# apple/ml-hugs

Hardware: AMD Instinct MI355X
Metric: rasterizer fwd+bwd FPS @1080p vs #Gaussians; achieved HBM GB/s vs peak (higher is better)
Workload: dtype f32

## Files before the change

### ml-hugs_amd/csrc/blend.hip

```cpp
#include <cstdlib>

#include "hgs_common.h"
#include "blend_fwd.h"

namespace hgs {

__global__ void __launch_bounds__(256)
blend_forward_kernel(Camera cam, uint32_t lastg, const uint2* __restrict__ ranges, const uint64_t* __restrict__ act,
                     size_t act_stride, const uint32_t* __restrict__ act_count, const Splat* __restrict__ splats, const float* __restrict__ bg, float* __restrict__ out_color,
                     float* __restrict__ final_T, uint32_t* __restrict__ n_contrib, const uint32_t* __restrict__ n_total,
                     int clamp_output, const uint32_t* __restrict__ large_tiles, uint32_t num_workers, int long_sorted, Ckpt ck)
{
    __shared__ DeepShared deep;
    if (((const_u32p)n_total)[1]) return;
    const uint32_t deep_min = num_workers != 0u ? ((const_u32p)n_total)[8] : 0u;
    const bool deep_blend = deep_min != 0u;
    if (blockIdx.x < num_workers) {
        if (deep_blend)
            deep_forward_worker(blockIdx.x, num_workers, cam, lastg, ranges, act, act_stride, act_count, splats, bg, out_color, final_T,
                                n_contrib, clamp_output, ck, large_tiles, n_total, deep, gridDim.x == num_workers);
        if (gridDim.x != num_workers) return;
        const uint32_t count = ((const_u32p)n_total)[2], threshold = ((const_u32p)n_total)[4];
        const int w = __builtin_amdgcn_readfirstlane(threadIdx.x >> 6);
        for (uint32_t li = blockIdx.x; li < count; li += num_workers) {
            const uint32_t tile = ((const_u32p)large_tiles)[li];
            const v2u range = ((const_u2p)ranges)[tile];
            const uint32_t n_tile = range.y - range.x;
            if (n_tile <= threshold || (deep_blend && n_tile > deep_min)) continue;
            float4* ck_tile = ckpt_begin(ck, tile, n_tile);
            blend_forward_wave(cam, lastg, (int)(tile % (uint32_t)cam.gx), (int)(tile / (uint32_t)cam.gx), w,
                               ((const_u32p)act_count)[tile * NUM_LISTS + w], act + (size_t)w * act_stride + range.x, splats, bg, out_color,
                               final_T, n_contrib, clamp_output, ck_tile, ck.quad_nproc + tile * 4u + (uint32_t)w);
        }
        return;
    }
    const int w = __builtin_amdgcn_readfirstlane(threadIdx.x >> 6);
    const int tile = (int)(blockIdx.x - num_workers);
    const v2u range = ((const_u2p)ranges)[tile];
    const uint32_t n_tile = range.y > range.x ? range.y - range.x : 0u;
    if (n_tile > ((const_u32p)n_total)[4]) {
        if (!long_sorted) return;
        if (deep_blend && n_tile > deep_min) {
            ckpt_begin(ck, (uint32_t)tile, n_tile);
            return;
        }
    }
    else if (long_sorted == 2) return;
    const uint32_t n = n_tile ? ((const_u32p)act_count)[tile * NUM_LISTS + w] : 0u;
    float4* ck_tile = ckpt_begin(ck, (uint32_t)tile, n_tile);
    blend_forward_wave(cam, lastg, tile % cam.gx, tile / cam.gx, w, n, act + (size_t)w * act_stride + range.x, splats, bg, out_color,
                       final_T, n_contrib, clamp_output, ck_tile, ck.quad_nproc + (uint32_t)tile * 4u + (uint32_t)w);
}

void launch_blend_forward(const Camera& cam, int P, const uint2* ranges, const uint64_t* act, size_t act_stride,
                          const uint32_t* act_count, const Splat* splats, const float* bg, float* out_color,
                          float* final_T, uint32_t* n_contrib, const uint32_t* n_total, bool clamp_output,
                          const uint32_t* large_tiles, bool all_tiles, bool long_sorted, const Ckpt& ck, hipStream_t st)
{
    const int tiles = cam.gx * cam.gy;
    const bool deep = deep_forward_enabled();
    const uint32_t workers = long_sorted && deep ? deep_workers_for(tiles) : 0u;
    if (!all_tiles && !deep) {
        hipLaunchKernelGGL(blend_forward_kernel, dim3(tiles), dim3(256), 0, st, cam, (uint32_t)(P - 1), ranges, act, act_stride, act_count,
                           splats, bg, out_color, final_T, n_contrib, n_total, clamp_output ? 1 : 0, large_tiles, 0u, 2, ck);
        return;
    }
    if (workers + (all_tiles ? tiles : 0) == 0) return;
    hipLaunchKernelGGL(blend_forward_kernel, dim3(workers + (all_tiles ? tiles : 0)), dim3(256), 0, st, cam, (uint32_t)(P - 1),
                       ranges, act, act_stride, act_count, splats, bg, out_color, final_T, n_contrib, n_total, clamp_output ? 1 : 0,
                       large_tiles, workers, long_sorted ? 1 : 0, ck);
}

template <int CTRL>
__device__ __forceinline__ float dpp_mov(float v)
{
    return __builtin_bit_cast(float, __builtin_amdgcn_update_dpp(0, __builtin_bit_cast(int, v), CTRL, 0xf, 0xf, true));
}
constexpr int DPP_QUAD_XOR1 = 0xB1;
constexpr int DPP_QUAD_XOR2 = 0x4E;
constexpr int DPP_ROW_ROR8 = 0x128;
constexpr int DPP_ROW_MIRROR = 0x140;
constexpr int DPP_ROW_HALF_MIRROR = 0x141;

typedef uint32_t swap_pair_t __attribute__((ext_vector_type(2)));
template <int W>
__device__ __forceinline__ float swap_add(float a, float b)
{
    const uint32_t ua = __builtin_bit_cast(uint32_t, a), ub = __builtin_bit_cast(uint32_t, b);
    swap_pair_t r;
    if constexpr (W == 32) r = __builtin_amdgcn_permlane32_swap(ua, ub, false, false);
    else r = __builtin_amdgcn_permlane16_swap(ua, ub, false, false);
    const uint32_t r0 = r.x, r1 = r.y;
    return __builtin_bit_cast(float, r0) + __builtin_bit_cast(float, r1);
}

template <int CTRL>
__device__ __forceinline__ float pair_step(float a, float b, bool hi)
{
    const float keep = hi ? b : a, send = hi ? a : b;
    return keep + dpp_mov<CTRL>(send);
}

struct PixBwd {
    float pxf, pyf;
    float T;
    float S;
    float g0, g1, g2;
    uint32_t last_contributor;
};

__device__ __forceinline__ unsigned long long bwd_pixel(const SplatRec& s, uint32_t pos1, PixBwd& p, float dy, float bdy,
                                                        float q, float (&v)[9])
{
    const float dx = s.x - p.pxf;
    const float t = __builtin_fmaf(s.A, dx, bdy);
    const float e = __builtin_fmaf(-t, t, q);
    const float alpha_uncapped = __builtin_amdgcn_exp2f(e);
    const float alpha = fminf(ALPHA_MAX, alpha_uncapped);
    float alpha_if_reached = pos1 <= p.last_contributor ? alpha : 0.0f;
    asm("" : "+v"(alpha_if_reached));
    const bool act_lane = alpha_if_reached >= ALPHA_MIN;
    const unsigned long long took = __builtin_amdgcn_ballot_w64(act_lane);
    if (act_lane) {
        const float inv = __builtin_amdgcn_rcpf(1.0f - alpha);
        p.T = p.T * inv;
        const float cg = __builtin_fmaf(s.r, p.g0, __builtin_fmaf(s.g, p.g1, s.b * p.g2));
        const float dL_dalpha = __builtin_fmaf(p.T, cg, -(p.S * inv));
        const float dch = alpha * p.T;
        p.S = __builtin_fmaf(cg, dch, p.S);
        const float u = alpha_uncapped * dL_dalpha;
        const float ux = u * dx, uy = u * dy;
        v[0] += ux;
        v[1] += uy;
        v[2] = __builtin_fmaf(ux, dx, v[2]);
        v[3] = __builtin_fmaf(ux, dy, v[3]);
        v[4] = __builtin_fmaf(uy, dy, v[4]);
        v[5] += u;
        v[6] = __builtin_fmaf(dch, p.g0, v[6]);
        v[7] = __builtin_fmaf(dch, p.g1, v[7]);
        v[8] = __builtin_fmaf(dch, p.g2, v[8]);
    }
    return took;
}

struct BwdSegment {
    uint32_t lo, hi;
    const float4* start;
    const float4* end_state;
};

template <int NQ, bool SEG = false>
__device__ __forceinline__ void
blend_backward_wave(const Camera& cam, uint32_t lastg, int tile, int w, v2u range, const uint64_t* __restrict__ act,
                    size_t act_stride, const uint32_t* __restrict__ act_count, const Splat* __restrict__ splats,
                    const float* __restrict__ bg, const float* __restrict__ final_T, const uint32_t* __restrict__ n_contrib,
                    const float* __restrict__ dL_dpix, float* __restrict__ grad_accum, const BwdSegment seg = BwdSegment{})
{
    static_assert(!SEG || NQ == 1, "segments are per quad");
    const int lane = threadIdx.x & 63;
    const int tx = tile % cam.gx, ty = tile / cam.gx;
    const int list_id = NQ == 4 ? 4 : w;
    const size_t HW = (size_t)cam.H * cam.W;
    const float bg0 = bg[0], bg1 = bg[1], bg2 = bg[2];

    PixBwd p[NQ];
    uint32_t wmax = 0;
    float ld_T[NQ], ld_g[NQ][3];
    uint32_t ld_n[NQ];
    bool in_img[NQ];
#pragma unroll
    for (int k = 0; k < NQ; ++k) {
        const int quad = NQ == 4 ? k : w;
        const int px = tx * TILE + (quad & 1) * 8 + (lane & 7);
        const int py = ty * TILE + (quad >> 1) * 8 + (lane >> 3);
        in_img[k] = px < cam.W && py < cam.H;
        const size_t pix = in_img[k] ? (size_t)py * cam.W + px : 0;
        p[k].pxf = (float)px, p[k].pyf = (float)py;
        ld_T[k] = final_T[pix], ld_n[k] = n_contrib[pix];
        ld_g[k][0] = dL_dpix[pix], ld_g[k][1] = dL_dpix[HW + pix], ld_g[k][2] = dL_dpix[2 * HW + pix];
    }
    float4 ck_start = make_float4(0.f, 0.f, 0.f, 0.f), ck_end = ck_start;
    if (SEG && seg.start) ck_start = seg.start[lane], ck_end = seg.end_state[lane];
#pragma unroll
    for (int k = 0; k < NQ; ++k) {
        const float Tf = in_img[k] ? ld_T[k] : 0.0f;
        p[k].T = Tf;
        p[k].g0 = in_img[k] && (ld_n[k] >> 29 & 1u) ? ld_g[k][0] : 0.0f;
        p[k].g1 = in_img[k] && (ld_n[k] >> 30 & 1u) ? ld_g[k][1] : 0.0f;
        p[k].g2 = in_img[k] && (ld_n[k] >> 31 & 1u) ? ld_g[k][2] : 0.0f;
        p[k].S = Tf * (bg0 * p[k].g0 + bg1 * p[k].g1 + bg2 * p[k].g2);
        if (SEG && seg.start) {
            p[k].T = __builtin_fabsf(ck_start.x);
            p[k].S = __builtin_fmaf(p[k].g0, ck_end.y - ck_start.y,
                                    __builtin_fmaf(p[k].g1, ck_end.z - ck_start.z, __builtin_fmaf(p[k].g2, ck_end.w - ck_start.w, p[k].S)));
        }
        p[k].last_contributor = in_img[k] ? (ld_n[k] & 0x0FFFFFFFu) : 0u;
        wmax = max(wmax, p[k].last_contributor);
    }
#pragma unroll
    for (int d = 32; d >= 1; d >>= 1) wmax = max(wmax, (uint32_t)__shfl_xor((int)wmax, d, 64));
    wmax = __builtin_amdgcn_readfirstlane(wmax);
    if (wmax == 0) return;
    const bool b3 = lane & 8;
    const int half_row = lane >> 3;
    const int slot_in_row[4] = {0, 2, 1, 3};
    const int slot_of_lane = lane == 63 ? 8 : ((lane & 7) == 0 ? slot_in_row[half_row >> 1] + 4 * (half_row & 1) : -1);

    uint32_t n = SEG ? seg.hi - seg.lo : ((const_u32p)act_count)[tile * NUM_LISTS + list_id];
    if (n == 0) return;
    const uint64_t* first = act + (size_t)list_id * act_stride + range.x + (SEG ? seg.lo : 0u);
    if (SEG && (uint32_t)(((const_u64p)first)[0] >> 32) > wmax) return;
    if ((uint32_t)(((const_u64p)first)[n - 1] >> 32) > wmax) {
        uint32_t lo = 0, hi = n - 1;
        while (lo < hi) {
            const uint32_t mid = (lo + hi) >> 1;
            if ((uint32_t)(((const_u64p)first)[mid] >> 32) <= wmax) lo = mid + 1; else hi = mid;
        }
        n = lo;
        if (n == 0) return;
    }
    const uint64_t* top = first + n;

    auto backward_entry = [&](const SplatRec& s, uint32_t val, uint32_t pos1) {
        if (pos1 > wmax) return;
        float v[9] = {0.f, 0.f, 0.f, 0.f, 0.f, 0.f, 0.f, 0.f, 0.f};
        unsigned long long took = 0ull;
        if constexpr (NQ == 4) {
#pragma unroll
            for (int r = 0; r < 2; ++r) {
                if (((val >> (GID_BITS + 2 * r)) & 3u) == 0u) continue;
                const float dy = s.y - p[2 * r].pyf, bdy = s.B * dy, cdy = s.C * dy, q = __builtin_fmaf(-cdy, cdy, s.L);
                if ((val >> (GID_BITS + 2 * r)) & 1u) took |= bwd_pixel(s, pos1, p[2 * r], dy, bdy, q, v);
                if ((val >> (GID_BITS + 2 * r + 1)) & 1u) took |= bwd_pixel(s, pos1, p[2 * r + 1], dy, bdy, q, v);
            }
        } else {
            const float dy = s.y - p[0].pyf, bdy = s.B * dy, cdy = s.C * dy, q = __builtin_fmaf(-cdy, cdy, s.L);
            took = bwd_pixel(s, pos1, p[0], dy, bdy, q, v);
        }
        if (took == 0ull) return;
        const float s0 = swap_add<32>(v[0], v[1]), s1 = swap_add<32>(v[2], v[3]);
        const float s2 = swap_add<32>(v[4], v[5]), s3 = swap_add<32>(v[6], v[7]);
        const float t0 = swap_add<16>(s0, s1), t1 = swap_add<16>(s2, s3);
        float y = pair_step<DPP_ROW_ROR8>(t0, t1, b3);
        y += dpp_mov<DPP_ROW_HALF_MIRROR>(y);
        y += dpp_mov<DPP_QUAD_XOR2>(y);
        y += dpp_mov<DPP_QUAD_XOR1>(y);
        float vb = v[8] + dpp_mov<DPP_QUAD_XOR1>(v[8]);
        vb += dpp_mov<DPP_QUAD_XOR2>(vb);
        vb += dpp_mov<DPP_ROW_HALF_MIRROR>(vb);
        vb += dpp_mov<DPP_ROW_MIRROR>(vb);
        asm("s_nop 1\n\tv_add_f32_dpp %0, %0, %0 row_bcast:15 row_mask:0xa bank_mask:0xf" : "+v"(vb));
        asm("s_nop 1\n\tv_add_f32_dpp %0, %0, %0 row_bcast:31 row_mask:0xc bank_mask:0xf" : "+v"(vb));
        if (slot_of_lane >= 0) atomicAdd(grad_accum + (size_t)(val & GID_MASK) * 12u + slot_of_lane, lane == 63 ? vb : y);
    };

    v4u eA = load_pair(top - 2, 0);
    SplatRec rA0 = load_rec(splats, eA.z, lastg), rA1 = load_rec(splats, eA.x, lastg);
    v4u eB = load_pair(top - 4, 0);
    for (uint32_t j = 0; j < n; j += 4) {
        __builtin_amdgcn_s_waitcnt(0xC07F);
        const SplatRec rB0 = load_rec(splats, eB.z, lastg), rB1 = load_rec(splats, eB.x, lastg);
        const v4u eA2 = load_pair(top - 6 - j, 0);
        backward_entry(rA0, eA.z, eA.w);
        if (j + 1 < n) backward_entry(rA1, eA.x, eA.y);
        if (j + 2 >= n) break;
        rA0 = load_rec(splats, eA2.z, lastg), rA1 = load_rec(splats, eA2.x, lastg);
        const v4u eB2 = load_pair(top - 8 - j, 0);
        backward_entry(rB0, eB.z, eB.w);
        if (j + 3 < n) backward_entry(rB1, eB.x, eB.y);
        eA = eA2, eB = eB2;
    }
}

template <int NQ>
__global__ void __launch_bounds__(256)
blend_backward_kernel(Camera cam, uint32_t lastg, const uint2* __restrict__ ranges, const uint64_t* __restrict__ act,
                      size_t act_stride, const uint32_t* __restrict__ act_count, const Splat* __restrict__ splats,
                      const float* __restrict__ bg, const float* __restrict__ final_T, const uint32_t* __restrict__ n_contrib,
                      const float* __restrict__ dL_dpix, float* __restrict__ grad_accum, uint32_t skip_from)
{
    const int num_tiles = cam.gx * cam.gy;
    const int w = __builtin_amdgcn_readfirstlane(threadIdx.x >> 6);
    const int vbid = NQ == 1 ? (int)blockIdx.x : (int)blockIdx.x * 4 + w;
    if (vbid >= num_tiles) return;
    const int tile = vbid;
    const v2u range = ((const_u2p)ranges)[tile];
    if (range.y <= range.x) return;
    if (skip_from && range.y - range.x >= skip_from) return;
    blend_backward_wave<NQ>(cam, lastg, tile, w, range, act, act_stride, act_count, splats, bg, final_T, n_contrib, dL_dpix, grad_accum);
}

__device__ __forceinline__ void
blend_backward_slot(uint32_t slot, const Camera& cam, uint32_t lastg, const uint2* __restrict__ ranges, const uint64_t* __restrict__ act,
                    size_t act_stride, const Splat* __restrict__ splats, const float* __restrict__ bg, const float* __restrict__ final_T,
                    const uint32_t* __restrict__ n_contrib, const float* __restrict__ dL_dpix, float* __restrict__ grad_accum, const Ckpt& ck)
{
    const int w = __builtin_amdgcn_readfirstlane(threadIdx.x >> 6);
    if (slot >= ((const_u32p)ck.seg_first)[cam.gx * cam.gy]) return;
    const uint32_t tile = ((const_u32p)ck.slot_tile)[slot];
    if (tile == CKPT_SLOT_NONE) return;
    const uint32_t first_slot = ((const_u32p)ck.seg_first)[tile];
    const uint32_t m = slot - first_slot;
    const uint32_t walked = ((const_u32p)ck.quad_nproc)[tile * 4u + (uint32_t)w];
    const uint32_t segs = (walked + (uint32_t)(CKPT_SEG - 1)) >> CKPT_SHIFT;
    if (m >= segs) return;
    const v2u range = ((const_u2p)ranges)[tile];
    BwdSegment seg;
    seg.lo = m << CKPT_SHIFT, seg.hi = min(walked, (m + 1u) << CKPT_SHIFT);
    seg.start = m + 1u < segs ? ck.state + (size_t)(first_slot + m) * 256u + w * 64 : nullptr;
    seg.end_state = ck.state + (size_t)(first_slot + segs - 1u) * 256u + w * 64;
    blend_backward_wave<1, true>(cam, lastg, (int)tile, w, range, act, act_stride, nullptr, splats, bg, final_T, n_contrib, dL_dpix,
                                 grad_accum, seg);
}

__global__ void __launch_bounds__(256)
blend_backward_segmented_kernel(Camera cam, uint32_t lastg, const uint2* __restrict__ ranges, const uint64_t* __restrict__ act,
                                size_t act_stride, const Splat* __restrict__ splats, const float* __restrict__ bg,
                                const float* __restrict__ final_T, const uint32_t* __restrict__ n_contrib,
                                const float* __restrict__ dL_dpix, float* __restrict__ grad_accum, Ckpt ck)
{
    blend_backward_slot(blockIdx.x, cam, lastg, ranges, act, act_stride, splats, bg, final_T, n_contrib, dL_dpix, grad_accum, ck);
}

#ifndef HGS_MIXED_ATTR
#define HGS_MIXED_ATTR
#endif
__global__ void __launch_bounds__(256) HGS_MIXED_ATTR
blend_backward_mixed_kernel(Camera cam, uint32_t lastg, const uint2* __restrict__ ranges, const uint64_t* __restrict__ act,
                            size_t act_stride, const uint32_t* __restrict__ act_count, const Splat* __restrict__ splats,
                            const float* __restrict__ bg, const float* __restrict__ final_T, const uint32_t* __restrict__ n_contrib,
                            const float* __restrict__ dL_dpix, float* __restrict__ grad_accum, Ckpt ck, uint32_t dense_blocks)
{
    if (blockIdx.x >= dense_blocks) {
        blend_backward_slot(blockIdx.x - dense_blocks, cam, lastg, ranges, act, act_stride, splats, bg, final_T, n_contrib, dL_dpix,
                            grad_accum, ck);
        return;
    }
    const int w = __builtin_amdgcn_readfirstlane(threadIdx.x >> 6);
    const int tile = (int)blockIdx.x * 4 + w;
    if (tile >= cam.gx * cam.gy) return;
    const v2u range = ((const_u2p)ranges)[tile];
    if (range.y <= range.x || range.y - range.x >= CKPT_DEEP_MIN) return;
    blend_backward_wave<4>(cam, lastg, tile, w, range, act, act_stride, act_count, splats, bg, final_T, n_contrib, dL_dpix, grad_accum);
}

void launch_blend_backward(const Camera& cam, int P, const uint2* ranges, const uint64_t* act, size_t act_stride,
                           const uint32_t* act_count, bool sparse_frame, const Splat* splats, const float* bg,
                           const float* final_T, const uint32_t* n_contrib, const float* dL_dpix, float* grad_accum,
                           const Ckpt& ck, int64_t num_rendered, int64_t dense_slots, hipStream_t st)
{
    const int num_tiles = cam.gx * cam.gy;
    const int force = switches().bwd_waves_per_tile;
    const bool per_quad = force ? force == 4 : sparse_frame;
    if (ck.state) {
        uint32_t slots = (uint32_t)(num_rendered >> CKPT_SHIFT) + (uint32_t)num_tiles;
        if (!sparse_frame && dense_slots >= 0 && (uint64_t)dense_slots < slots) slots = (uint32_t)dense_slots;
        const bool two_launches = switches().bwd_two_launches;
        if ((sparse_frame || two_launches) && slots)
            hipLaunchKernelGGL(blend_backward_segmented_kernel, dim3(slots), dim3(256), 0, st, cam, (uint32_t)(P - 1), ranges, act,
                               act_stride, splats, bg, final_T, n_contrib, dL_dpix, grad_accum, ck);
        if (!sparse_frame && two_launches)
            hipLaunchKernelGGL(blend_backward_kernel<4>, dim3((num_tiles + 3) / 4), dim3(256), 0, st, cam, (uint32_t)(P - 1), ranges,
                               act, act_stride, act_count, splats, bg, final_T, n_contrib, dL_dpix, grad_accum, CKPT_DEEP_MIN);
        else if (!sparse_frame) {
            const uint32_t dense_blocks = (uint32_t)(num_tiles + 3) / 4u;
            hipLaunchKernelGGL(blend_backward_mixed_kernel, dim3(dense_blocks + slots), dim3(256), 0, st, cam, (uint32_t)(P - 1), ranges,
                               act, act_stride, act_count, splats, bg, final_T, n_contrib, dL_dpix, grad_accum, ck, dense_blocks);
        }
    } else if (per_quad)
        hipLaunchKernelGGL(blend_backward_kernel<1>, dim3(num_tiles), dim3(256), 0, st, cam, (uint32_t)(P - 1), ranges, act,
                           act_stride, act_count, splats, bg, final_T, n_contrib, dL_dpix, grad_accum, 0u);
    else
        hipLaunchKernelGGL(blend_backward_kernel<4>, dim3((num_tiles + 3) / 4), dim3(256), 0, st, cam, (uint32_t)(P - 1), ranges,
                           act, act_stride, act_count, splats, bg, final_T, n_contrib, dL_dpix, grad_accum, 0u);
}

}
```

Measured before the change: 2126.

## Replace permlane/DPP gradient reduction with per-wave LDS transpose reduction

Each backward entry now writes its eight per-lane gradient partials into a per-wave LDS buffer and reads them back transposed as two float4s, then finishes with three DPP steps. This replaces the earlier permlane32/16 swap-and-DPP butterfly. Two splats are staged into separate buffers before reading, so their reductions can interleave. The change adds 16 KB of shared memory per block plus wave barriers and fences, which may reduce occupancy and adds LDS traffic.

```diff
diff --git a/ml-hugs_amd/csrc/blend.hip b/ml-hugs_amd/csrc/blend.hip
--- a/ml-hugs_amd/csrc/blend.hip
+++ b/ml-hugs_amd/csrc/blend.hip
@@ -78,28 +78,10 @@
 }
 constexpr int DPP_QUAD_XOR1 = 0xB1;
 constexpr int DPP_QUAD_XOR2 = 0x4E;
-constexpr int DPP_ROW_ROR8 = 0x128;
 constexpr int DPP_ROW_MIRROR = 0x140;
 constexpr int DPP_ROW_HALF_MIRROR = 0x141;
 
-typedef uint32_t swap_pair_t __attribute__((ext_vector_type(2)));
-template <int W>
-__device__ __forceinline__ float swap_add(float a, float b)
-{
-    const uint32_t ua = __builtin_bit_cast(uint32_t, a), ub = __builtin_bit_cast(uint32_t, b);
-    swap_pair_t r;
-    if constexpr (W == 32) r = __builtin_amdgcn_permlane32_swap(ua, ub, false, false);
-    else r = __builtin_amdgcn_permlane16_swap(ua, ub, false, false);
-    const uint32_t r0 = r.x, r1 = r.y;
-    return __builtin_bit_cast(float, r0) + __builtin_bit_cast(float, r1);
-}
-
-template <int CTRL>
-__device__ __forceinline__ float pair_step(float a, float b, bool hi)
-{
-    const float keep = hi ? b : a, send = hi ? a : b;
-    return keep + dpp_mov<CTRL>(send);
-}
+constexpr int BWD_RED_FLOATS = 2 * 8 * 64;
 
 struct PixBwd {
     float pxf, pyf;
@@ -154,7 +136,8 @@
 blend_backward_wave(const Camera& cam, uint32_t lastg, int tile, int w, v2u range, const uint64_t* __restrict__ act,
                     size_t act_stride, const uint32_t* __restrict__ act_count, const Splat* __restrict__ splats,
                     const float* __restrict__ bg, const float* __restrict__ final_T, const uint32_t* __restrict__ n_contrib,
-                    const float* __restrict__ dL_dpix, float* __restrict__ grad_accum, const BwdSegment seg = BwdSegment{})
+                    const float* __restrict__ dL_dpix, float* __restrict__ grad_accum, float* red_all,
+                    const BwdSegment seg = BwdSegment{})
 {
     static_assert(!SEG || NQ == 1, "segments are per quad");
     const int lane = threadIdx.x & 63;
@@ -201,10 +184,10 @@
     for (int d = 32; d >= 1; d >>= 1) wmax = max(wmax, (uint32_t)__shfl_xor((int)wmax, d, 64));
     wmax = __builtin_amdgcn_readfirstlane(wmax);
     if (wmax == 0) return;
-    const bool b3 = lane & 8;
-    const int half_row = lane >> 3;
-    const int slot_in_row[4] = {0, 2, 1, 3};
-    const int slot_of_lane = lane == 63 ? 8 : ((lane & 7) == 0 ? slot_in_row[half_row >> 1] + 4 * (half_row & 1) : -1);
+    float* const red = red_all + w * BWD_RED_FLOATS;
+    const int grp = lane >> 3;
+    const int rd = grp * 64 + (lane & 7) * 8 + (grp & 1) * 4;
+    const int slot_of_lane = lane == 63 ? 8 : ((lane & 7) == 0 ? grp : -1);
 
     uint32_t n = SEG ? seg.hi - seg.lo : ((const_u32p)act_count)[tile * NUM_LISTS + list_id];
     if (n == 0) return;
@@ -221,8 +204,8 @@
     }
     const uint64_t* top = first + n;
 
-    auto backward_entry = [&](const SplatRec& s, uint32_t val, uint32_t pos1) {
-        if (pos1 > wmax) return;
+    auto backward_entry = [&](const SplatRec& s, uint32_t val, uint32_t pos1, int e, float& vb) -> bool {
+        if (pos1 > wmax) return false;
         float v[9] = {0.f, 0.f, 0.f, 0.f, 0.f, 0.f, 0.f, 0.f, 0.f};
         unsigned long long took = 0ull;
         if constexpr (NQ == 4) {
@@ -237,20 +220,31 @@
             const float dy = s.y - p[0].pyf, bdy = s.B * dy, cdy = s.C * dy, q = __builtin_fmaf(-cdy, cdy, s.L);
             took = bwd_pixel(s, pos1, p[0], dy, bdy, q, v);
         }
-        if (took == 0ull) return;
-        const float s0 = swap_add<32>(v[0], v[1]), s1 = swap_add<32>(v[2], v[3]);
-        const float s2 = swap_add<32>(v[4], v[5]), s3 = swap_add<32>(v[6], v[7]);
-        const float t0 = swap_add<16>(s0, s1), t1 = swap_add<16>(s2, s3);
-        float y = pair_step<DPP_ROW_ROR8>(t0, t1, b3);
-        y += dpp_mov<DPP_ROW_HALF_MIRROR>(y);
-        y += dpp_mov<DPP_QUAD_XOR2>(y);
-        y += dpp_mov<DPP_QUAD_XOR1>(y);
-        float vb = v[8] + dpp_mov<DPP_QUAD_XOR1>(v[8]);
+        if (took == 0ull) return false;
+        float* const buf = red + e * (8 * 64);
+#pragma unroll
+        for (int k = 0; k < 8; ++k) buf[k * 64 + lane] = v[k];
+        vb = v[8] + dpp_mov<DPP_QUAD_XOR1>(v[8]);
         vb += dpp_mov<DPP_QUAD_XOR2>(vb);
         vb += dpp_mov<DPP_ROW_HALF_MIRROR>(vb);
         vb += dpp_mov<DPP_ROW_MIRROR>(vb);
         asm("s_nop 1\n\tv_add_f32_dpp %0, %0, %0 row_bcast:15 row_mask:0xa bank_mask:0xf" : "+v"(vb));
         asm("s_nop 1\n\tv_add_f32_dpp %0, %0, %0 row_bcast:31 row_mask:0xc bank_mask:0xf" : "+v"(vb));
+        return true;
+    };
+    auto backward_read = [&](int e, float4& ra, float4& rb) {
+        const float* const buf = red + e * (8 * 64);
+        __builtin_amdgcn_fence(__ATOMIC_RELEASE, "wavefront");
+        __builtin_amdgcn_wave_barrier();
+        __builtin_amdgcn_fence(__ATOMIC_ACQUIRE, "wavefront");
+        ra = *(const float4*)(buf + rd);
+        rb = *(const float4*)(buf + (rd ^ 4));
+    };
+    auto backward_finish = [&](uint32_t val, const float4& ra, const float4& rb, float vb) {
+        float y = ((ra.x + ra.y) + (ra.z + ra.w)) + ((rb.x + rb.y) + (rb.z + rb.w));
+        y += dpp_mov<DPP_QUAD_XOR1>(y);
+        y += dpp_mov<DPP_QUAD_XOR2>(y);
+        y += dpp_mov<DPP_ROW_HALF_MIRROR>(y);
         if (slot_of_lane >= 0) atomicAdd(grad_accum + (size_t)(val & GID_MASK) * 12u + slot_of_lane, lane == 63 ? vb : y);
     };
 
@@ -261,13 +255,19 @@
         __builtin_amdgcn_s_waitcnt(0xC07F);
         const SplatRec rB0 = load_rec(splats, eB.z, lastg), rB1 = load_rec(splats, eB.x, lastg);
         const v4u eA2 = load_pair(top - 6 - j, 0);
-        backward_entry(rA0, eA.z, eA.w);
-        if (j + 1 < n) backward_entry(rA1, eA.x, eA.y);
+        float4 r00, r01, r10, r11;
+        float vb0, vb1;
+        const bool tA0 = backward_entry(rA0, eA.z, eA.w, 0, vb0);
+        const bool tA1 = j + 1 < n && backward_entry(rA1, eA.x, eA.y, 1, vb1);
+        if (tA0) backward_read(0, r00, r01), backward_finish(eA.z, r00, r01, vb0);
+        if (tA1) backward_read(1, r10, r11), backward_finish(eA.x, r10, r11, vb1);
         if (j + 2 >= n) break;
         rA0 = load_rec(splats, eA2.z, lastg), rA1 = load_rec(splats, eA2.x, lastg);
         const v4u eB2 = load_pair(top - 8 - j, 0);
-        backward_entry(rB0, eB.z, eB.w);
-        if (j + 3 < n) backward_entry(rB1, eB.x, eB.y);
+        const bool tB0 = backward_entry(rB0, eB.z, eB.w, 0, vb0);
+        const bool tB1 = j + 3 < n && backward_entry(rB1, eB.x, eB.y, 1, vb1);
+        if (tB0) backward_read(0, r00, r01), backward_finish(eB.z, r00, r01, vb0);
+        if (tB1) backward_read(1, r10, r11), backward_finish(eB.x, r10, r11, vb1);
         eA = eA2, eB = eB2;
     }
 }
@@ -287,13 +287,16 @@
     const v2u range = ((const_u2p)ranges)[tile];
     if (range.y <= range.x) return;
     if (skip_from && range.y - range.x >= skip_from) return;
-    blend_backward_wave<NQ>(cam, lastg, tile, w, range, act, act_stride, act_count, splats, bg, final_T, n_contrib, dL_dpix, grad_accum);
+    __shared__ float red[4 * BWD_RED_FLOATS];
+    blend_backward_wave<NQ>(cam, lastg, tile, w, range, act, act_stride, act_count, splats, bg, final_T, n_contrib, dL_dpix, grad_accum,
+                            red);
 }
 
 __device__ __forceinline__ void
 blend_backward_slot(uint32_t slot, const Camera& cam, uint32_t lastg, const uint2* __restrict__ ranges, const uint64_t* __restrict__ act,
                     size_t act_stride, const Splat* __restrict__ splats, const float* __restrict__ bg, const float* __restrict__ final_T,
-                    const uint32_t* __restrict__ n_contrib, const float* __restrict__ dL_dpix, float* __restrict__ grad_accum, const Ckpt& ck)
+                    const uint32_t* __restrict__ n_contrib, const float* __restrict__ dL_dpix, float* __restrict__ grad_accum, const Ckpt& ck,
+                    float* red)
 {
     const int w = __builtin_amdgcn_readfirstlane(threadIdx.x >> 6);
     if (slot >= ((const_u32p)ck.seg_first)[cam.gx * cam.gy]) return;
@@ -310,7 +313,7 @@
     seg.start = m + 1u < segs ? ck.state + (size_t)(first_slot + m) * 256u + w * 64 : nullptr;
     seg.end_state = ck.state + (size_t)(first_slot + segs - 1u) * 256u + w * 64;
     blend_backward_wave<1, true>(cam, lastg, (int)tile, w, range, act, act_stride, nullptr, splats, bg, final_T, n_contrib, dL_dpix,
-                                 grad_accum, seg);
+                                 grad_accum, red, seg);
 }
 
 __global__ void __launch_bounds__(256)
@@ -319,7 +322,8 @@
                                 const float* __restrict__ final_T, const uint32_t* __restrict__ n_contrib,
                                 const float* __restrict__ dL_dpix, float* __restrict__ grad_accum, Ckpt ck)
 {
-    blend_backward_slot(blockIdx.x, cam, lastg, ranges, act, act_stride, splats, bg, final_T, n_contrib, dL_dpix, grad_accum, ck);
+    __shared__ float red[4 * BWD_RED_FLOATS];
+    blend_backward_slot(blockIdx.x, cam, lastg, ranges, act, act_stride, splats, bg, final_T, n_contrib, dL_dpix, grad_accum, ck, red);
 }
 
 #ifndef HGS_MIXED_ATTR
@@ -331,9 +335,10 @@
                             const float* __restrict__ bg, const float* __restrict__ final_T, const uint32_t* __restrict__ n_contrib,
                             const float* __restrict__ dL_dpix, float* __restrict__ grad_accum, Ckpt ck, uint32_t dense_blocks)
 {
+    __shared__ float red[4 * BWD_RED_FLOATS];
     if (blockIdx.x >= dense_blocks) {
         blend_backward_slot(blockIdx.x - dense_blocks, cam, lastg, ranges, act, act_stride, splats, bg, final_T, n_contrib, dL_dpix,
-                            grad_accum, ck);
+                            grad_accum, ck, red);
         return;
     }
     const int w = __builtin_amdgcn_readfirstlane(threadIdx.x >> 6);
@@ -341,7 +346,8 @@
     if (tile >= cam.gx * cam.gy) return;
     const v2u range = ((const_u2p)ranges)[tile];
     if (range.y <= range.x || range.y - range.x >= CKPT_DEEP_MIN) return;
-    blend_backward_wave<4>(cam, lastg, tile, w, range, act, act_stride, act_count, splats, bg, final_T, n_contrib, dL_dpix, grad_accum);
+    blend_backward_wave<4>(cam, lastg, tile, w, range, act, act_stride, act_count, splats, bg, final_T, n_contrib, dL_dpix, grad_accum,
+                           red);
 }
 
 void launch_blend_backward(const Camera& cam, int P, const uint2* ranges, const uint64_t* act, size_t act_stride,
```

Result: faster. 2245, median of 6 (+5.6%).
